# realphongha/UDP-Pose

Measured on AMD Instinct MI355X. Metric: images/sec HRNet-W32 256x192 (infer+decode), higher is better.
Workload: dtype f16x2 (split fp16 hi+lo operands = 22 bits, 3 fp16 MFMAs per product, fp32 accumulate); 1 GPU; w32 256x192 f16x2 inference, batch=64 per GPU, flip-test on, DARK decode (forward on 2N images + flip fuse + udp_decode_gaussian); global_batch=64, parallelism=replicas x1 (no data-path collective), weights=seeded synthetic, BN stats calibrated (tests/golden/bn_calib_w32_gaussian.npz)

## Files before the change

udp-pose_amd/csrc/conv_ws.hip:

```cpp
#include "conv_dev.h"

namespace udp {

template <int NB>
struct ResH2 {
  u32x4 hi[NB / 2], lo[NB / 2];
};
template <int NB>
__device__ __forceinline__ void load_res_h2(ResH2<NB>& o, __amdgpu_buffer_rsrc_t r, unsigned voff, unsigned lo_off) {
#pragma unroll
  for (int h = 0; h < NB / 2; ++h) {
    o.hi[h] = __builtin_amdgcn_raw_buffer_load_b128(r, voff + 16 * h, 0, UDP_H2_RES_AUX);
    o.lo[h] = __builtin_amdgcn_raw_buffer_load_b128(r, voff + lo_off + 16 * h, 0, UDP_H2_RES_AUX);
  }
}
template <int NB>
__device__ __forceinline__ void add_res_h2(f32x4 (&v)[NB], const ResH2<NB>& o) {
#pragma unroll
  for (int h = 0; h < NB / 2; ++h) h2_add8(v[2 * h], v[2 * h + 1], __builtin_bit_cast(f16x8, o.hi[h]), __builtin_bit_cast(f16x8, o.lo[h]));
}

template <int KS, int STRIDE, int PB, int CP, bool NCHW, bool OUT2 = false, int HS = 0>
__device__ __forceinline__ void conv_ws_body(const ConvParams& p, const int tile_id, const int cby) {
  using T = H2;
  constexpr int CK = 32, ESZ = 2, NB = 2, NW = 4;
  constexpr int PAD = KS / 2, TAPS = KS * KS;
  extern __shared__ __attribute__((aligned(16))) unsigned char smem[];

  UDP_STAMP(0);
  const int tid = threadIdx.x;
  const int lane = tid & 63;
  const int wave = __builtin_amdgcn_readfirstlane(tid >> 6);
  const int li = lane & 15;
  const int kg = lane >> 4;
  const int cp = wave % CP, pg = wave / CP;

  int t = tile_id;
  const int tx = t % p.tiles_x;
  t /= p.tiles_x;
  const int ty = t % p.tiles_y;
  const int n0 = (t / p.tiles_y) * p.G;
  const int y0 = ty * p.R;
  const int x0 = tx * p.TW;

  const int IH = p.IH, IW = p.IW;
  const int npix_in = p.G * IH * IW;
  const int in_groups = (npix_in + 15) >> 4;
  const int in_bytes = in_groups * 16 * ROWB;
  const int stage_bytes = 2 * in_bytes;
  const int nchunks = (p.Cin + CK - 1) / CK;
  const bool ragged = (p.Cin % CK) != 0;
  const int RT = p.R * p.TW;
  const int M = p.G * RT;
  const unsigned inpb = (unsigned)p.in_pitch * ESZ * 2;
  const unsigned outpb = (unsigned)p.out_pitch * ESZ * 2, respb = (unsigned)p.res_pitch * ESZ * 2;
  const unsigned in_lo = (unsigned)p.in_pitch * ESZ;
  const unsigned out_lo = (unsigned)p.out_pitch * ESZ, res_lo = (unsigned)p.res_pitch * ESZ;

  const unsigned out_pix = (unsigned)p.N * p.Hout * p.Wout;
  const __amdgpu_buffer_rsrc_t r_in = __builtin_amdgcn_make_buffer_rsrc(
      const_cast<void*>(p.in), 0, (unsigned)p.N * p.Hin * p.Win * inpb, 0x00020000);
  const unsigned npairs = (unsigned)p.CoutPad >> 5;
  const __amdgpu_buffer_rsrc_t r_w = __builtin_amdgcn_make_buffer_rsrc(
      const_cast<void*>(p.wgt), 0, (unsigned)TAPS * nchunks * npairs * 4096u, 0x00020000);
#if UDP_WS_DBG & 32
  const bool dbg_nost = nchunks == 1;
#else
  constexpr bool dbg_nost = false;
#endif
#if UDP_WS_DBG & 64
  const bool dbg_nores = nchunks == 1;
#else
  constexpr bool dbg_nores = false;
#endif
  const __amdgpu_buffer_rsrc_t r_out = __builtin_amdgcn_make_buffer_rsrc(
      p.out, 0, (!p.out || dbg_nost) ? 0 : NCHW ? out_pix * p.Cout * 4 : out_pix * outpb, 0x00020000);
  const __amdgpu_buffer_rsrc_t r_bias = __builtin_amdgcn_make_buffer_rsrc(
      const_cast<float*>(p.bias), 0, (unsigned)p.CoutPad * 4u, 0x00020000);
  const __amdgpu_buffer_rsrc_t r_res = __builtin_amdgcn_make_buffer_rsrc(
      const_cast<void*>(p.res), 0, (p.res && !dbg_nores) ? out_pix * respb : 0, 0x00020000);

  const int cwave = (cby * CP + cp) * 32;
  const int cbase = cwave + 8 * kg;
  const unsigned wvoff = (unsigned)lane * 16u;
  const unsigned wpair = (unsigned)(cby * CP + cp) * 4096u;
  constexpr int AD = UDP_WS_AD;
  f16x8 ah[AD][NB], al[AD][NB];
  const int nsteps = nchunks * TAPS;
  auto load_a = [&](int s, f16x8 (&h)[NB], f16x8 (&l)[NB]) __attribute__((always_inline)) {
    const int c = s / TAPS, tap = s - c * TAPS;
    const unsigned soff = (unsigned)(tap * nchunks + c) * (npairs * 4096u) + wpair;
#pragma unroll
    for (int nb = 0; nb < NB; ++nb) {
      h[nb] = __builtin_bit_cast(f16x8, __builtin_amdgcn_raw_buffer_load_b128(r_w, wvoff + 2048u * nb, soff, 0));
      l[nb] = __builtin_bit_cast(f16x8, __builtin_amdgcn_raw_buffer_load_b128(r_w, wvoff + 2048u * nb + 1024u, soff, 0));
    }
  };

#pragma unroll
  for (int k = 0; k < AD - 1; ++k) load_a(k < nsteps ? k : nsteps - 1, ah[k], al[k]);
  f32x4 bias[NB];
#pragma unroll
  for (int nb = 0; nb < NB; ++nb)
    bias[nb] = __builtin_bit_cast(f32x4, __builtin_amdgcn_raw_buffer_load_b128(r_bias, (unsigned)(cbase + 4 * nb) * 4u, 0, 0));

  const int srow = lane >> 2, spart = lane & 3;
  const int gy0 = y0 * STRIDE - PAD, gx0 = x0 * STRIDE - PAD;
  unsigned src_off[MAXG];
#pragma unroll
  for (int i = 0; i < MAXG; ++i) {
    unsigned off = kOobOff;
    if ((wave + NW * i) * 16 < npix_in) {
      const int row = (wave + NW * i) * 16 + srow;
      const int tmp = fdiv20(row, p.mIW);
      const int ix = row - (int)__umul24(tmp, IW);
      const int g = fdiv20(tmp, p.mIH);
      const int iy = tmp - (int)__umul24(g, IH);
      const int n = n0 + g, gy = gy0 + iy, gx = gx0 + ix;
      const bool ok = row < npix_in && n < p.N && (unsigned)gy < (unsigned)p.Hin && (unsigned)gx < (unsigned)p.Win;
      const unsigned pix = __umul24(__umul24(n, p.Hin) + gy, p.Win) + gx;
      off = ok ? pix * inpb + p.in_coff * ESZ + ((spart ^ swz<T>(row)) << 4) : kOobOff;
    }
    src_off[i] = off;
  }
  auto stage = [&](int c, unsigned char* sb) __attribute__((always_inline)) {
    const unsigned coff = (unsigned)c * (CK * ESZ);
    const bool cut = ragged && c == nchunks - 1;
    const int parts_left = (p.Cin - c * CK) / 8;
#pragma unroll
    for (int i = 0; i < MAXG; ++i) {
      const int gidx = wave + NW * i;
      if (gidx < in_groups) {
        unsigned off = src_off[i] + coff;
        if (cut && (spart ^ swz<T>(gidx * 16 + srow)) >= parts_left) off = kOobOff;
        blds16(r_in, off, sb + gidx * (16 * ROWB));
        blds16(r_in, off + in_lo, sb + in_bytes + gidx * (16 * ROWB));
      }
    }
  };

  UDP_STAMP(1);
  stage(0, smem);

  int prow[PB], opix[PB], ocrd[PB];
#pragma unroll
  for (int i = 0; i < PB; ++i) {
    const int m0 = (pg * PB + i) * 16 + li;
    const int m = m0 < M ? m0 : M - 1;
    const int g = fdiv20(m, p.mRT);
    const int rem = m - (int)__umul24(g, RT);
    const int r = fdiv20(rem, p.mTW);
    const int x = rem - (int)__umul24(r, p.TW);
    prow[i] = (int)__umul24(__umul24(g, IH) + r * STRIDE, IW) + x * STRIDE;
    const int n = n0 + g, y = y0 + r, xo = x0 + x;
    const bool ok = m0 < M && n < p.N && y < p.Hout && xo < p.Wout && (NCHW || cbase < p.Cout);
    const unsigned pix = __umul24(__umul24(n, p.Hout) + y, p.Wout) + xo;
    opix[i] = ok ? (int)pix : -1;
    ocrd[i] = ok ? (y | (xo << 10) | (n << 20)) : -1;
  }

  const float winv = __builtin_ldexpf(1.f, -p.wexp);
  f32x4 acc[PB][NB];
#pragma unroll
  for (int i = 0; i < PB; ++i)
#pragma unroll
    for (int nb = 0; nb < NB; ++nb) acc[i][nb] = f32x4{0.f, 0.f, 0.f, 0.f};

  constexpr int NR = NCHW ? 0 : PB * NB;
  ResH2<NB> rres[NCHW ? 1 : PB];
  __builtin_amdgcn_sched_barrier(0);
  asm volatile("" ::: "memory");
  if constexpr (!NCHW) {
#pragma unroll
    for (int i = 0; i < PB; ++i)
      load_res_h2(rres[i], r_res, opix[i] >= 0 ? (unsigned)opix[i] * respb + (p.res_coff + cbase) * ESZ : kOobOff, res_lo);
  }
  asm volatile("" ::: "memory");
  __builtin_amdgcn_sched_barrier(0);

  UDP_STAMP(2);
  int c = 0, tap = 0;
  const unsigned char* sb = smem;
  auto step = [&](auto BUFC, int s) __attribute__((always_inline)) {
    constexpr int BUF = decltype(BUFC)::value;
#if !(UDP_WS_DBG & 1)
    load_a(s + AD - 1 < nsteps ? s + AD - 1 : nsteps - 1, ah[(BUF + AD - 1) % AD], al[(BUF + AD - 1) % AD]);
#endif
    if (tap == 0) {
      if (c == 1) UDP_STAMP(9);
      if (c == 2) UDP_STAMP(11);
      if (c == 4) UDP_STAMP(13);
      bool refill = false;
      if constexpr (STRIDE == 2 || OUT2) refill = p.sbuf && c > 0;
      if (refill) {
        __syncthreads();
        stage(c, smem);
        asm volatile("s_waitcnt vmcnt(0)" ::: "memory");
        __syncthreads();
        sb = smem;
      } else {
        if (s == 0)
          asm volatile("s_waitcnt vmcnt(%0)" ::"n"(2 * NB + NR) : "memory");
        else
          asm volatile("s_waitcnt vmcnt(%0)" ::"n"(2 * NB) : "memory");
        if (s == 0) UDP_STAMP(3);
        __syncthreads();
        if (s == 0) UDP_STAMP(4);
        if (c == 1) UDP_STAMP(10);
        if (c == 2) UDP_STAMP(12);
        if (c == 4) UDP_STAMP(14);
#if !(UDP_WS_DBG & 4)
        if (c + 1 < nchunks && !((STRIDE == 2 || OUT2) && p.sbuf)) stage(c + 1, smem + ((c + 1) & 1) * stage_bytes);
#endif
        sb = smem + (c & 1) * stage_bytes;
      }
    }
    f16x8 a2[NB];
#pragma unroll
    for (int nb = 0; nb < NB; ++nb) a2[nb] = ah[BUF][nb] * (_Float16)0x1p-11f;
    const int tap_rows = KS == 1 ? 0 : (tap / KS) * IW + tap % KS;
    f16x8 xh[3], xl[3];
    auto load_b = [&](int i, f16x8& h, f16x8& l) __attribute__((always_inline)) {
      const int row = prow[i] + tap_rows;
      const unsigned char* q = sb + row * ROWB + ((kg ^ swz<T>(row)) << 4);
      h = *reinterpret_cast<const f16x8*>(q);
      l = *reinterpret_cast<const f16x8*>(q + in_bytes);
    };
    load_b(0, xh[0], xl[0]);
    if (PB > 1) load_b(1, xh[1], xl[1]);
#pragma unroll
    for (int i = 0; i < PB; ++i) {
#if !(UDP_WS_DBG & 2)
      if (i + 2 < PB) load_b(i + 2, xh[(i + 2) % 3], xl[(i + 2) % 3]);
#endif
      __builtin_amdgcn_sched_barrier(0);
#if UDP_WS_DBG & 16
      acc[i][0] = __builtin_amdgcn_mfma_f32_16x16x32_f16(ah[BUF][0] + al[BUF][1] + a2[0] + a2[1], xh[i % 3] + xl[i % 3], acc[i][0], 0, 0, 0);
#else
#pragma unroll
      for (int nb = 0; nb < NB; ++nb) acc[i][nb] = __builtin_amdgcn_mfma_f32_16x16x32_f16(ah[BUF][nb], xh[i % 3], acc[i][nb], 0, 0, 0);
#pragma unroll
      for (int nb = 0; nb < NB; ++nb) acc[i][nb] = __builtin_amdgcn_mfma_f32_16x16x32_f16(al[BUF][nb], xh[i % 3], acc[i][nb], 0, 0, 0);
#pragma unroll
      for (int nb = 0; nb < NB; ++nb) acc[i][nb] = __builtin_amdgcn_mfma_f32_16x16x32_f16(a2[nb], xl[i % 3], acc[i][nb], 0, 0, 0);
#endif
    }
    if (++tap == TAPS) {
      tap = 0;
      ++c;
    }
  };
  for (int s = 0; s < nsteps; s += AD) {
    step(std::integral_constant<int, 0>{}, s);
    if (s + 1 < nsteps) step(std::integral_constant<int, 1>{}, s + 1);
    if (s + 2 < nsteps) step(std::integral_constant<int, 2>{}, s + 2);
    if constexpr (AD > 3) if (s + 3 < nsteps) step(std::integral_constant<int, 3>{}, s + 3);
    if constexpr (AD > 4) if (s + 4 < nsteps) step(std::integral_constant<int, 4>{}, s + 4);
    if constexpr (AD > 5) if (s + 5 < nsteps) step(std::integral_constant<int, 5>{}, s + 5);
  }
  UDP_STAMP(5);
#pragma unroll
  for (int i = 0; i < PB; ++i) {
#pragma unroll
    for (int nb = 0; nb < NB; ++nb)
#pragma unroll
      for (int q = 0; q < 4; ++q) acc[i][nb][q] = __builtin_fmaf(acc[i][nb][q], winv, bias[nb][q]);
    if constexpr (!NCHW) add_res_h2(acc[i], rres[i]);
  }

#pragma unroll
  for (int i = 0; i < PB; ++i) {
    f32x4 v[NB];
#pragma unroll
    for (int nb = 0; nb < NB; ++nb) v[nb] = acc[i][nb];
    if constexpr (NCHW) {
      const int crd = ocrd[i];
      const int y = crd & 1023, xo = (crd >> 10) & 1023, n = crd >> 20;
      const unsigned hw = __umul24(p.Hout, p.Wout);
      const unsigned base = __umul24(__umul24(__umul24(n, p.Cout), p.Hout) + y, p.Wout) + xo;
#pragma unroll
      for (int nb = 0; nb < NB; ++nb)
#pragma unroll
        for (int q = 0; q < 4; ++q) {
          const int cc = cbase + 4 * nb + q;
          float f = v[nb][q];
          if (p.relu) f = f > 0.f ? f : 0.f;
          const unsigned off = (crd >= 0 && cc < p.Cout) ? (base + cc * hw) * 4u : kOobOff;
          __builtin_amdgcn_raw_buffer_store_b32(__builtin_bit_cast(unsigned, f), r_out, off, 0, 0);
        }
    } else {
      const unsigned ooff = opix[i] >= 0 ? (unsigned)opix[i] * outpb + (p.out_coff + cbase) * ESZ : kOobOff;
      if (p.nup) {
        const int crd = ocrd[i];
        const int y = crd & 1023, xo = (crd >> 10) & 1023, n = crd >> 20;
#pragma unroll
        for (int u = 0; u < 3; ++u) {
          if (u < p.nup) {
            const int sh = p.up_shift[u];
            const long up_pix = ((long)(n * (p.Hout >> sh) + (y >> sh)) * (p.Wout >> sh) + (xo >> sh));
            if (crd >= 0)
              add_vec<T, NB>(v, reinterpret_cast<const unsigned char*>(p.up[u]) + (up_pix * p.Cout * 2 + cbase) * ESZ, p.Cout * ESZ);
          }
        }
      }
      if constexpr (HS) {
#pragma unroll
        for (int nb = 0; nb < NB; ++nb)
#pragma unroll
          for (int q = 0; q < 4; ++q) v[nb][q] = act_hs<HS>(v[nb][q]);
      } else
      if (p.relu) {
#pragma unroll
        for (int nb = 0; nb < NB; ++nb)
#pragma unroll
          for (int q = 0; q < 4; ++q) v[nb][q] = v[nb][q] > 0.f ? v[nb][q] : 0.f;
      }
      store_vec_buf<T, NB>(r_out, ooff, out_lo, v);
      if (OUT2 && p.nout2) {
        f16x8 sh, sl;
        h2_split8(v[0], v[1], sh, sl);
        f32x4 vr[NB];
#pragma unroll
        for (int q = 0; q < 4; ++q) {
          vr[0][q] = (float)sh[q] + (float)sl[q] * kLoInv;
          vr[1][q] = (float)sh[4 + q] + (float)sl[4 + q] * kLoInv;
        }
#pragma unroll
        for (int u = 0; u < 2; ++u) {
          if (u < p.nout2 && opix[i] >= 0) {
            const size_t px = (size_t)opix[i];
            const _Float16* a = reinterpret_cast<const _Float16*>(p.add2[u]) + px * (2 * (size_t)p.add2_pitch[u]) + p.add2_coff[u] + cbase;
            const f16x8 ah8 = *reinterpret_cast<const f16x8*>(a), al8 = *reinterpret_cast<const f16x8*>(a + p.add2_pitch[u]);
            f32x4 w[NB];
#pragma unroll
            for (int q = 0; q < 4; ++q) {
              w[0][q] = ((float)ah8[q] + (float)al8[q] * kLoInv) + vr[0][q];
              w[1][q] = ((float)ah8[4 + q] + (float)al8[4 + q] * kLoInv) + vr[1][q];
            }
            f16x8 oh, ol;
            h2_split8(w[0], w[1], oh, ol);
            _Float16* o2 = reinterpret_cast<_Float16*>(p.out2[u]) + px * (2 * (size_t)p.out2_pitch[u]) + p.out2_coff[u] + cbase;
            *reinterpret_cast<f16x8*>(o2) = oh;
            *reinterpret_cast<f16x8*>(o2 + p.out2_pitch[u]) = ol;
          }
        }
      }
    }
  }
  UDP_STAMP(6);
#ifdef UDP_STAMPS
  asm volatile("s_waitcnt vmcnt(0)" ::: "memory");
  UDP_STAMP(7);
#endif
}

__host__ __device__ __forceinline__ void ws_decode(unsigned b, unsigned ntiles, unsigned nc, int& tile, int& cby) {
  if (nc == 1) {
    tile = (int)b;
    cby = 0;
    return;
  }
  const unsigned full = (ntiles >> 3) * 8u * nc;
  unsigned base = 0, width = 8, r = b;
  if (b < full) {
    const unsigned g = b / (8u * nc);
    r = b - g * 8u * nc;
    base = g * 8u;
  } else {
    r = b - full;
    base = (ntiles >> 3) * 8u;
    width = ntiles & 7u;
  }
  const unsigned c = r / width;
  cby = (int)c;
  tile = (int)(base + r - c * width);
}

template <int KS, int STRIDE, int PB, int CP, bool NCHW>
__global__ __launch_bounds__(256, 2) void conv_ws_h2_kernel(const ConvParams p) {
  int tile, cby;
  ws_decode(blockIdx.x + gridDim.x * blockIdx.y, gridDim.x, gridDim.y, tile, cby);
  conv_ws_body<KS, STRIDE, PB, CP, NCHW, KS == 3 && STRIDE == 1 && !NCHW>(p, tile, cby);
}

template <int PB, int CP, int ACT>
__global__ __launch_bounds__(256, 2) void conv_ws_hs_kernel(const ConvParams p) {
  int tile, cby;
  ws_decode(blockIdx.x + gridDim.x * blockIdx.y, gridDim.x, gridDim.y, tile, cby);
  conv_ws_body<1, 1, PB, CP, false, false, ACT>(p, tile, cby);
}

#ifndef UDP_WS_MPB
#define UDP_WS_MPB 6
#define UDP_WS_MOCC 2
#endif
template <int KS>
__global__ __launch_bounds__(256, UDP_WS_MOCC) void conv_ws_multi(const ConvMulti m) {
  const unsigned b = blockIdx.x;
  int j, tile, cby;
  int code;
  const unsigned e = __builtin_amdgcn_readfirstlane(m.tab[(b >> 3) < (unsigned)kMultiTab ? (b >> 3) : 0u]);
  if (m.tab_n) {
    j = (int)(e & 3u);
    code = 1 << ((e >> 2) & 3u);
    cby = (int)((e >> 4) & 63u);
    tile = (int)((e >> 10) + (b & 7u));
  } else {
    int sg = 0;
#pragma unroll
    for (int k = 1; k < kMultiSegs; ++k) sg += b >= m.seg_start[k];
    j = __builtin_amdgcn_readfirstlane(m.seg_mem[sg]);
    const unsigned r = __builtin_amdgcn_readfirstlane(b - m.seg_start[sg] + m.seg_first[sg]);
    ws_decode(r, m.tiles[j], m.ncby[j], tile, cby);
    tile = __builtin_amdgcn_readfirstlane(tile);
    cby = __builtin_amdgcn_readfirstlane(cby);
    code = m.code[j];
  }
  switch (code) {
    case 1: conv_ws_body<KS, 1, UDP_WS_MPB, 1, false>(m.p[j], tile, (int)cby); break;
    case 2: conv_ws_body<KS, 1, UDP_WS_MPB, 2, false>(m.p[j], tile, (int)cby); break;
    default: conv_ws_body<KS, 1, UDP_WS_MPB, 4, false>(m.p[j], tile, (int)cby); break;
  }
}

template <int KS, int STRIDE, int PB, int CP, bool NCHW>
static int describe_ws_one(const ConvParams& p, size_t lds, Launch* out) {
  static bool attr_set = false;
  const void* kern = reinterpret_cast<const void*>(&conv_ws_h2_kernel<KS, STRIDE, PB, CP, NCHW>);
  if (!attr_set) {
    UDP_HIP_CHECK(hipFuncSetAttribute(kern, hipFuncAttributeMaxDynamicSharedMemorySize, 160 * 1024));
    attr_set = true;
  }
  out->fn = kern;
  out->grid = dim3(p.ntiles, p.CoutPad / (CP * 32));
  out->block = dim3(256);
  out->lds = (unsigned)lds;
  out->p = p;
  return UDP_OK;
}
template <int KS, int STRIDE, bool NCHW>
static int describe_ws_pb(const ConvParams& p, int pb, int cp, size_t lds, Launch* out) {
#define UDP_WS(B, C) \
  if (pb == B && cp == C) return describe_ws_one<KS, STRIDE, B, C, NCHW>(p, lds, out);
  UDP_WS(2, 1) UDP_WS(3, 1) UDP_WS(4, 1) UDP_WS(6, 1) UDP_WS(2, 2) UDP_WS(3, 2) UDP_WS(4, 2) UDP_WS(6, 2)
  UDP_WS(2, 4) UDP_WS(3, 4) UDP_WS(4, 4) UDP_WS(6, 4)
#undef UDP_WS
  return 1;
}
template <int PB, int CP, int ACT>
static int describe_ws_hs_one(const ConvParams& p, size_t lds, Launch* out) {
  static bool attr_set = false;
  const void* kern = reinterpret_cast<const void*>(&conv_ws_hs_kernel<PB, CP, ACT>);
  if (!attr_set) {
    UDP_HIP_CHECK(hipFuncSetAttribute(kern, hipFuncAttributeMaxDynamicSharedMemorySize, 160 * 1024));
    attr_set = true;
  }
  out->fn = kern;
  out->grid = dim3(p.ntiles, p.CoutPad / (CP * 32));
  out->block = dim3(256);
  out->lds = (unsigned)lds;
  out->p = p;
  return UDP_OK;
}
static int describe_ws_hs(const ConvParams& p, int pb, int cp, size_t lds, Launch* out) {
#define UDP_WS(B, C) \
  if (pb == B && cp == C) return p.relu == UDP_ACT_SILU ? describe_ws_hs_one<B, C, UDP_ACT_SILU>(p, lds, out) : describe_ws_hs_one<B, C, UDP_ACT_HSWISH>(p, lds, out);
  UDP_WS(2, 1) UDP_WS(3, 1) UDP_WS(4, 1) UDP_WS(6, 1) UDP_WS(2, 2) UDP_WS(3, 2) UDP_WS(4, 2) UDP_WS(6, 2)
  UDP_WS(2, 4) UDP_WS(3, 4) UDP_WS(4, 4) UDP_WS(6, 4)
#undef UDP_WS
  return 1;
}
struct WsTile {
  int cp, pb, G, R, TW, wgs, sbuf;
  size_t lds;
};
static bool ws_tile(const ConvParams& p, int ks, int stride, int cp, int pb, WsTile* t, bool own_launch) {
  const int pg = 4 / cp;
  const int maxM = 16 * pb * pg;
  bool have = false;
  double best_util = 0.0;
  for (int split = 1; split <= 4 || !have; ++split) {
    if (split > 8) break;
    const int TW = ceil_div(p.Wout, split);
    if (TW > 64 || TW > maxM || (have && TW < 8)) continue;
    int maxR = maxM / TW;
    if (maxR > p.Hout) maxR = p.Hout;
    int R = largest_divisor_leq(p.Hout, maxR);
    if (R * 2 <= maxR) R = maxR;
    int G = 1;
    if (R == p.Hout && TW == p.Wout) {
      G = maxM / (R * TW);
      if (G > p.N) G = p.N;
      if (G < 1) G = 1;
    }
    auto npix = [&](int g, int r) { return g * ((r - 1) * stride + ks) * ((TW - 1) * stride + ks); };
    while (npix(G, R) > MAXG * 64 && G > 1) --G;
    while (npix(G, R) > MAXG * 64 && R > 1) R = (R + 1) / 2;
    if (npix(G, R) > MAXG * 64) continue;
    int nstage = ceil_div(p.Cin, 32) > 1 ? 2 : 1;
    size_t lds = (size_t)((npix(G, R) + 15) / 16) * 16 * ROWB * 2 * nstage;
    static const int sbuf_mode = getenv("UDP_POSE_WS_SBUF") == nullptr ? 1 : atoi(getenv("UDP_POSE_WS_SBUF"));
    const bool sbuf_kernel = stride == 2 || (ks == 3 && own_launch && sbuf_mode != 2);
    const bool sbuf = sbuf_kernel && nstage == 2 && lds > 80 * 1024 && lds / 2 <= 80 * 1024 && sbuf_mode != 0;
    if (sbuf) {
      nstage = 1;
      lds /= 2;
    }
    if (lds > 160 * 1024) continue;
    const int need = ceil_div(ceil_div(G * R * TW, 16), pg);
    if (need > pb) continue;
    const int pbe = need <= 2 ? 2 : need <= 3 ? 3 : need <= 4 ? 4 : 6;
    const int tiles = ceil_div(p.N, G) * ceil_div(p.Hout, R) * ceil_div(p.Wout, TW);
    const double util = (double)p.N * p.Hout * p.Wout / ((double)tiles * 16 * pbe * pg) *
                        ((double)G * R * TW * stride * stride / (double)npix(G, R));
    if (!have || util > best_util + 0.05) {
      have = true;
      best_util = util;
      t->cp = cp;
      t->pb = pbe;
      t->G = G;
      t->R = R;
      t->TW = TW;
      t->lds = lds;
      t->sbuf = sbuf ? 1 : 0;
      t->wgs = tiles * (p.CoutPad / (cp * 32));
    }
  }
  return have;
}

static long g_ws_fill_wgs = 512;
void ws_set_fill_wgs(long wgs) { g_ws_fill_wgs = wgs; }

int describe_conv_ws(ConvParams p, int ks, int stride, Launch* out, bool grouped) {
  if (p.relu >= UDP_ACT_HSWISH && (ks != 1 || stride != 1 || p.out_nchw_f32 || p.res || p.nup || p.nout2 || grouped))
    return fail(UDP_ERR_UNSUPPORTED, "hard-swish / SiLU (activation codes 2, 4): plain 1x1 stride-1 NHWC convs on their own launch only");
  if ((stride != 1 && stride != 2) || (ks != 3 && ks != 1) || (p.out_nchw_f32 && stride != 1))
    return fail(UDP_ERR_UNSUPPORTED, "fragment-major weights (wfmt 1): conv ks=%d stride=%d nchw_out=%d has no weight-stationary kernel",
                ks, stride, p.out_nchw_f32);
  auto knob = [](const char* name, long dflt) {
    const char* v = getenv(name);
    return v ? atol(v) : dflt;
  };
  const int pairs = p.CoutPad / 32;
  const int force_cp = (int)knob("UDP_POSE_WS_CP", 0), force_pb = (int)knob("UDP_POSE_WS_PB", 0);
  const long min_wgs = grouped ? 0 : knob("UDP_POSE_WS_MINWGS", g_ws_fill_wgs);
  WsTile best{}, t{};
  bool have = false;
  for (int pb : {6, 4, 3, 2}) {
    for (int cp : {4, 2, 1}) {
      if (pairs % cp || (force_cp && cp != force_cp) || (force_pb && pb != force_pb)) continue;
      if (grouped && stride == 1 && UDP_WS_MPB != 6 && pb != UDP_WS_MPB) continue;
      if (!ws_tile(p, ks, stride, cp, pb, &t, !grouped && !p.out_nchw_f32)) continue;
      const bool fills = t.wgs >= min_wgs, best_fills = have && best.wgs >= min_wgs;
      if (!have || (!best_fills && (fills || t.wgs > best.wgs))) {
        best = t;
        have = true;
      }
    }
  }
  if (!have) return fail(UDP_ERR_UNSUPPORTED, "weight-stationary conv: no tile for %dx%d C%d->%d", p.Hout, p.Wout, p.Cin, p.Cout);
  p.G = best.G;
  p.R = best.R;
  p.TW = best.TW;
  p.sbuf = best.sbuf;
  p.IH = (p.R - 1) * stride + ks;
  p.IW = (p.TW - 1) * stride + ks;
  p.tiles_x = ceil_div(p.Wout, p.TW);
  p.tiles_y = ceil_div(p.Hout, p.R);
  auto magic = [](int d) { return (unsigned)(((1u << 20) + (unsigned)d - 1) / (unsigned)d); };
  p.mIW = magic(p.IW);
  p.mIH = magic(p.IH);
  p.mRT = magic(p.R * p.TW);
  p.mTW = magic(p.TW);
  p.ntiles = ceil_div(p.N, p.G) * p.tiles_y * p.tiles_x;
  if (getenv("UDP_POSE_DEBUG_TILES"))
    fprintf(stderr, "ws conv k%d s%d %dx%d C%d->%d: G=%d R=%d TW=%d CP=%d PB=%d lds=%zu%s wgs=%d\n", ks, stride, p.Hout, p.Wout, p.Cin,
            p.Cout, p.G, p.R, p.TW, best.cp, best.pb, best.lds, best.sbuf ? " (one stage buffer)" : "", best.wgs);
  int rc = 1;
  if (ks == 3 && stride == 1 && !p.out_nchw_f32) rc = describe_ws_pb<3, 1, false>(p, best.pb, best.cp, best.lds, out);
  if (ks == 3 && stride == 1 && p.out_nchw_f32) rc = describe_ws_pb<3, 1, true>(p, best.pb, best.cp, best.lds, out);
  if (ks == 3 && stride == 2) rc = describe_ws_pb<3, 2, false>(p, best.pb, best.cp, best.lds, out);
  if (ks == 1 && stride == 1 && !p.out_nchw_f32)
    rc = p.relu >= UDP_ACT_HSWISH ? describe_ws_hs(p, best.pb, best.cp, best.lds, out) : describe_ws_pb<1, 1, false>(p, best.pb, best.cp, best.lds, out);
  if (ks == 1 && stride == 1 && p.out_nchw_f32) rc = describe_ws_pb<1, 1, true>(p, best.pb, best.cp, best.lds, out);
  if (ks == 1 && stride == 2) rc = describe_ws_pb<1, 2, false>(p, best.pb, best.cp, best.lds, out);
  if (rc == 1) return fail(UDP_ERR_UNSUPPORTED, "weight-stationary conv: no kernel for PB=%d CP=%d", best.pb, best.cp);
  if (rc == UDP_OK && p.nout2 && !(ks == 3 && stride == 1))
    return fail(UDP_ERR_UNSUPPORTED, "second outputs: 3x3 stride-1 convs only");
  if (rc == UDP_OK && grouped && best.pb == UDP_WS_MPB && stride == 1 && !p.nout2) {
    out->groupable = 300 + ks * 10 + 6;
    out->ws_cp = best.cp;
  }
  return rc;
}

static void ws_order(ConvMulti* m, int n) {
  struct Seg {
    unsigned start, first, cnt;
    int mem;
  };
  unsigned cnt_of[4];
  unsigned total = 0;
  for (int j = 0; j < n; ++j) {
    cnt_of[j] = (j + 1 < n ? m->start[j + 1] : m->start[4]) - m->start[j];
    total += cnt_of[j];
  }
  const char* mode = getenv("UDP_POSE_WS_ORDER");
  const bool lpt = mode && strcmp(mode, "lpt") == 0;
  const unsigned bias = getenv("UDP_POSE_WS_BIAS") ? (unsigned)atoi(getenv("UDP_POSE_WS_BIAS")) : 125u;
  auto build = [&](unsigned g) {
    std::vector<Seg> segs;
    unsigned lo[4] = {0, 0, 0, 0};
    unsigned at = 0;
    auto take = [&](int j, unsigned cnt) {
      if (cnt > cnt_of[j] - lo[j]) cnt = cnt_of[j] - lo[j];
      if (!cnt) return;
      if (!segs.empty() && segs.back().mem == j && segs.back().first + segs.back().cnt == lo[j])
        segs.back().cnt += cnt;
      else
        segs.push_back({at, lo[j], cnt, j});
      lo[j] += cnt;
      at += cnt;
    };
    if (!lpt) {
      const unsigned nb = cnt_of[n - 1];
      const unsigned na = total - nb;
      unsigned ta = 0, tb = 0;
      while (ta < na && tb < nb) {
        if ((unsigned long long)ta * nb * 100ull <= (unsigned long long)tb * na * bias) {
          int j = 0;
          while (lo[j] == cnt_of[j]) ++j;
          const unsigned c = cnt_of[j] - lo[j] < g ? cnt_of[j] - lo[j] : g;
          take(j, c);
          ta += c;
        } else {
          const unsigned c = nb - tb < g ? nb - tb : g;
          take(n - 1, c);
          tb += c;
        }
      }
    }
    for (int j = 0; j < n; ++j) take(j, cnt_of[j] - lo[j]);
    return segs;
  };
  unsigned g = getenv("UDP_POSE_WS_G") ? (unsigned)atoi(getenv("UDP_POSE_WS_G")) : 32u;
  if (g < 8 || g % 8) g = 32;
  std::vector<Seg> segs = build(g);
  m->tab_n = 0;
  bool ok = total % 8 == 0 && total / 8 <= (unsigned)kMultiTab && getenv("UDP_POSE_WS_NOTAB") == nullptr;
  for (int j = 0; j < n && ok; ++j)
    ok = m->tiles[j] % 8 == 0 && m->ncby[j] <= 64 && m->tiles[j] < (1u << 22) && (m->code[j] == 1 || m->code[j] == 2 || m->code[j] == 4);
  for (size_t k = 0; k < segs.size() && ok; ++k) ok = segs[k].start % 8 == 0 && segs[k].first % 8 == 0;
  if (ok) {
    for (const Seg& sg : segs) {
      const int j = sg.mem;
      for (unsigned b = sg.start; b < sg.start + sg.cnt; b += 8) {
        int tile, cby;
        ws_decode(b - sg.start + sg.first, m->tiles[j], m->ncby[j], tile, cby);
        const unsigned cl = m->code[j] == 1 ? 0u : m->code[j] == 2 ? 1u : 2u;
        m->tab[b >> 3] = (unsigned)j | (cl << 2) | ((unsigned)cby << 4) | ((unsigned)tile << 10);
      }
    }
    m->tab_n = total / 8;
  }
  while (segs.size() > (size_t)kMultiSegs) {
    g += 8;
    segs = build(g);
  }
  for (int k = 0; k < kMultiSegs; ++k) {
    const bool have = (size_t)k < segs.size();
    m->seg_start[k] = have ? segs[k].start : 0xFFFFFFFFu;
    m->seg_first[k] = have ? segs[k].first : 0;
    m->seg_mem[k] = have ? segs[k].mem : 0;
  }
}

extern "C" int udp_debug_multi_order(const unsigned* tiles, const unsigned* ncby, const int* code, int n, unsigned cap,
                                     unsigned* out_member, unsigned* out_tile, unsigned* out_cby, int* used_table) {
  if (!tiles || !ncby || !code || n < 1 || n > 4 || !out_member || !out_tile || !out_cby) return -1;
  static ConvMulti m;
  memset(&m, 0, sizeof(m));
  unsigned total = 0;
  for (int j = 0; j < n; ++j) {
    m.start[j] = total;
    m.tiles[j] = tiles[j];
    m.ncby[j] = ncby[j];
    m.code[j] = code[j];
    total += tiles[j] * ncby[j];
  }
  for (int j = n; j < 5; ++j) m.start[j] = j < 4 ? 0xFFFFFFFFu : total;
  m.start[4] = total;
  for (int j = n; j < 4; ++j) m.tiles[j] = m.ncby[j] = 1;
  if (total > cap) return -1;
  ws_order(&m, n);
  if (used_table) *used_table = m.tab_n != 0;
  for (unsigned b = 0; b < total; ++b) {
    int j, tile, cby;
    if (m.tab_n) {
      const unsigned e = m.tab[b >> 3];
      j = (int)(e & 3u);
      if ((1 << ((e >> 2) & 3u)) != m.code[j]) return -1;
      cby = (int)((e >> 4) & 63u);
      tile = (int)((e >> 10) + (b & 7u));
    } else {
      int sg = 0;
      for (int k = 1; k < kMultiSegs; ++k) sg += b >= m.seg_start[k];
      j = m.seg_mem[sg];
      ws_decode(b - m.seg_start[sg] + m.seg_first[sg], m.tiles[j], m.ncby[j], tile, cby);
    }
    out_member[b] = (unsigned)j;
    out_tile[b] = (unsigned)tile;
    out_cby[b] = (unsigned)cby;
  }
  return (int)total;
}

int describe_ws_multi(const Launch* members, int n, ConvMulti* m, Launch* out) {
  static bool ws_attr_set = false;
  const void* wk[2] = {reinterpret_cast<const void*>(&conv_ws_multi<3>), reinterpret_cast<const void*>(&conv_ws_multi<1>)};
  if (!ws_attr_set) {
    for (const void* k : wk) UDP_HIP_CHECK(hipFuncSetAttribute(k, hipFuncAttributeMaxDynamicSharedMemorySize, 160 * 1024));
    ws_attr_set = true;
  }
  memset(m, 0, sizeof(*m));
  unsigned total = 0, lds = 0;
  for (int j = 0; j < n; ++j) {
    if (members[j].groupable != members[0].groupable) return fail(UDP_ERR_ARG, "describe_multi: mixed weight-stationary members");
    m->p[j] = members[j].p;
    m->start[j] = total;
    m->tiles[j] = members[j].grid.x;
    m->ncby[j] = members[j].grid.y;
    m->code[j] = members[j].ws_cp;
    total += members[j].grid.x * members[j].grid.y;
    if (members[j].lds > lds) lds = members[j].lds;
  }
  for (int j = n; j < 5; ++j) m->start[j] = j < 4 ? 0xFFFFFFFFu : total;
  for (int j = n; j < 4; ++j) m->tiles[j] = m->ncby[j] = 1;
  ws_order(m, n);
  out->fn = wk[members[0].groupable / 10 % 10 == 3 ? 0 : 1];
  out->grid = dim3(total);
  out->block = dim3(256);
  out->lds = lds;
  out->groupable = 0;
  return UDP_OK;
}

#ifdef UDP_STAMPS
int ws_set_stamps(unsigned long long* dev_buf) {
  UDP_HIP_CHECK(hipMemcpyToSymbol(HIP_SYMBOL(g_stamps), &dev_buf, sizeof(dev_buf)));
  return UDP_OK;
}
extern "C" int udp_debug_set_stamps_ws(unsigned long long* dev_buf) { return ws_set_stamps(dev_buf); }
#endif

template <int NCH, int PB, int RD, bool LDSW>
__global__ __launch_bounds__(LDSW ? 512 : 256) __attribute__((amdgpu_waves_per_eu(2))) void conv_chain_kernel(const ConvParams p) {
  using T = H2;
  constexpr int ESZ = 2, NB = 2, Q = 2;
  constexpr int NWAVES = LDSW ? 8 : 4;
  constexpr int AD = LDSW ? 2 : 3;
  extern __shared__ __attribute__((aligned(16))) unsigned char smem[];
  const int lane = threadIdx.x & 63, wave = __builtin_amdgcn_readfirstlane(threadIdx.x >> 6);
  const int li = lane & 15, kg = lane >> 4;
  const unsigned npix = (unsigned)p.N * p.Hout * p.Wout;
  constexpr int NP = 8;
  const int cout2 = p.up_shift[0];
  const unsigned inpb = (unsigned)p.in_pitch * ESZ * 2, outpb = (unsigned)p.out_pitch * ESZ * 2, respb = (unsigned)p.res_pitch * ESZ * 2;
  const unsigned zpb = (unsigned)cout2 * ESZ * 2;
  const unsigned in_lo = (unsigned)p.in_pitch * ESZ, out_lo = (unsigned)p.out_pitch * ESZ, res_lo = (unsigned)p.res_pitch * ESZ;
  const unsigned z_lo = (unsigned)cout2 * ESZ;
  const __amdgpu_buffer_rsrc_t r_in = __builtin_amdgcn_make_buffer_rsrc(const_cast<void*>(p.in), 0, (p.sbuf & 8) ? 0 : npix * inpb, 0x00020000);
  const __amdgpu_buffer_rsrc_t r_w = __builtin_amdgcn_make_buffer_rsrc(const_cast<void*>(p.wgt), 0, (p.sbuf & 1) ? 0 : (unsigned)NCH * NP * 4096u, 0x00020000);
  const __amdgpu_buffer_rsrc_t r_w2 = __builtin_amdgcn_make_buffer_rsrc(const_cast<void*>(p.wgt2), 0, (p.sbuf & 1) ? 0 : (unsigned)NP * Q * 4096u, 0x00020000);
  const __amdgpu_buffer_rsrc_t r_bias = __builtin_amdgcn_make_buffer_rsrc(const_cast<float*>(p.bias), 0, (unsigned)p.CoutPad * 4u, 0x00020000);
  const __amdgpu_buffer_rsrc_t r_bias2 = __builtin_amdgcn_make_buffer_rsrc(const_cast<float*>(p.bias2), 0, (unsigned)cout2 * 4u, 0x00020000);
  const __amdgpu_buffer_rsrc_t r_res = __builtin_amdgcn_make_buffer_rsrc(const_cast<void*>(p.res), 0, (p.res && !(p.sbuf & 4)) ? npix * respb : 0, 0x00020000);
  const __amdgpu_buffer_rsrc_t r_out = __builtin_amdgcn_make_buffer_rsrc(p.out, 0, (p.sbuf & 2) ? 0 : npix * outpb, 0x00020000);
  const __amdgpu_buffer_rsrc_t r_z = __builtin_amdgcn_make_buffer_rsrc(const_cast<void*>(p.up[0]), 0, (p.sbuf & 2) ? 0 : npix * zpb, 0x00020000);
  const float winv = __builtin_ldexpf(1.f, -p.wexp), winv2 = __builtin_ldexpf(1.f, -p.up_shift[1]);
  const unsigned wvoff = (unsigned)lane * 16u;

  constexpr unsigned kW1 = (unsigned)NCH * 8 * 4096u, kBias = kW1 + 8u * Q * 4096u;
  if constexpr (LDSW) {
    for (unsigned blk = wave; blk < kBias / 1024u; blk += NWAVES) {
      const bool first = blk * 1024u < kW1;
      blds16(first ? r_w : r_w2, (first ? blk * 1024u : blk * 1024u - kW1) + wvoff, smem + blk * 1024u);
    }
    float* sbias = reinterpret_cast<float*>(smem + kBias);
    if (threadIdx.x < 256 + 64) sbias[threadIdx.x] = threadIdx.x < 256 ? p.bias[threadIdx.x] : p.bias2[threadIdx.x - 256];
    asm volatile("s_waitcnt vmcnt(0)" ::: "memory");
    __syncthreads();
  }
  const unsigned ngroups = (npix + PB * 16 - 1) / (PB * 16);
  for (unsigned grp = (unsigned)blockIdx.x * NWAVES + wave; grp < ngroups; grp += LDSW ? gridDim.x * NWAVES : ngroups) {
  unsigned wv = wvoff;
  int kgl = kg;
  if constexpr (LDSW) {
    asm volatile("" : "+v"(wv));
    asm volatile("" : "+v"(kgl));
  }
  unsigned pix[PB];
  bool ok[PB];
#pragma unroll
  for (int i = 0; i < PB; ++i) {
    pix[i] = grp * (PB * 16) + i * 16 + li;
    ok[i] = pix[i] < npix;
  }
  f16x8 xh[PB][NCH], xl[PB][NCH];
#pragma unroll
  for (int i = 0; i < PB; ++i)
#pragma unroll
    for (int c = 0; c < NCH; ++c) {
      const unsigned off = ok[i] ? pix[i] * inpb + (unsigned)(p.in_coff + 32 * c + 8 * kgl) * ESZ : kOobOff;
      xh[i][c] = __builtin_bit_cast(f16x8, __builtin_amdgcn_raw_buffer_load_b128(r_in, off, 0, 0));
      xl[i][c] = __builtin_bit_cast(f16x8, __builtin_amdgcn_raw_buffer_load_b128(r_in, off + in_lo, 0, 0));
    }
  constexpr int S = NCH + Q;
  f16x8 ah[AD][NB], al[AD][NB];
  auto load_a = [&](int pr, int st, f16x8 (&h)[NB], f16x8 (&l)[NB]) __attribute__((always_inline)) {
    const bool first = st < NCH;
    const unsigned soff = first ? (unsigned)(st * NP + pr) * 4096u : (unsigned)(pr * Q + (st - NCH)) * 4096u;
#pragma unroll
    for (int nb = 0; nb < NB; ++nb) {
      if constexpr (LDSW) {
        const unsigned char* q = smem + (first ? 0u : kW1) + soff + wv + 2048u * nb;
        h[nb] = *reinterpret_cast<const f16x8*>(q);
        l[nb] = *reinterpret_cast<const f16x8*>(q + 1024);
      } else {
        h[nb] = __builtin_bit_cast(f16x8, __builtin_amdgcn_raw_buffer_load_b128(first ? r_w : r_w2, wv + 2048u * nb, soff, 0));
        l[nb] = __builtin_bit_cast(f16x8, __builtin_amdgcn_raw_buffer_load_b128(first ? r_w : r_w2, wv + 2048u * nb + 1024u, soff, 0));
      }
    }
  };
  ResH2<NB> rres[RD][PB];
  auto load_res = [&](int pr, ResH2<NB> (&r)[PB]) __attribute__((always_inline)) {
#pragma unroll
    for (int i = 0; i < PB; ++i)
      load_res_h2(r[i], r_res, ok[i] ? pix[i] * respb + (unsigned)(p.res_coff + 32 * pr + 8 * kgl) * ESZ : kOobOff, res_lo);
  };
#pragma unroll
  for (int k = 0; k < RD - 1; ++k) load_res(k, rres[k]);
  load_a(0, 0, ah[0], al[0]);
  if constexpr (AD > 2) load_a(0, 1, ah[1], al[1]);

  f32x4 acc2[PB][Q][NB];
#pragma unroll
  for (int i = 0; i < PB; ++i)
#pragma unroll
    for (int q = 0; q < Q; ++q)
#pragma unroll
      for (int nb = 0; nb < NB; ++nb) acc2[i][q][nb] = f32x4{0.f, 0.f, 0.f, 0.f};

  auto mfma3 = [&](f32x4 (&acc)[NB], const f16x8 (&h)[NB], const f16x8 (&l)[NB], const f16x8 (&a2)[NB], const f16x8 bh, const f16x8 bl)
      __attribute__((always_inline)) {
#pragma unroll
        for (int nb = 0; nb < NB; ++nb) acc[nb] = __builtin_amdgcn_mfma_f32_16x16x32_f16(h[nb], bh, acc[nb], 0, 0, 0);
#pragma unroll
        for (int nb = 0; nb < NB; ++nb) acc[nb] = __builtin_amdgcn_mfma_f32_16x16x32_f16(l[nb], bh, acc[nb], 0, 0, 0);
#pragma unroll
        for (int nb = 0; nb < NB; ++nb) acc[nb] = __builtin_amdgcn_mfma_f32_16x16x32_f16(a2[nb], bl, acc[nb], 0, 0, 0);
      };

  auto pair_body = [&](auto KC) __attribute__((always_inline)) {
    constexpr int pr = decltype(KC)::value, BUF0 = (pr * S) % AD, SIDE = pr % RD;
    if constexpr (pr + RD - 1 < NP) load_res(pr + RD - 1, rres[(SIDE + RD - 1) % RD]);
    f32x4 bias[NB];
#pragma unroll
    for (int nb = 0; nb < NB; ++nb) {
      if constexpr (LDSW)
        bias[nb] = *reinterpret_cast<const f32x4*>(smem + kBias + (unsigned)(32 * pr + 8 * kgl + 4 * nb) * 4u);
      else
        bias[nb] = __builtin_bit_cast(f32x4, __builtin_amdgcn_raw_buffer_load_b128(r_bias, (unsigned)(32 * pr + 8 * kgl + 4 * nb) * 4u, 0, 0));
    }
    f32x4 acc[PB][NB];
#pragma unroll
    for (int i = 0; i < PB; ++i)
#pragma unroll
      for (int nb = 0; nb < NB; ++nb) acc[i][nb] = f32x4{0.f, 0.f, 0.f, 0.f};
    f16x8 yh[PB], yl[PB];
#pragma unroll
    for (int st = 0; st < S; ++st) {
      constexpr int dummy = 0;
      (void)dummy;
      const int buf = (BUF0 + st) % AD;
      {
// ... 109 lines not shown
```

Measured before the change: 8117 images/s.

## Add PB=8 weight-stationary conv variant with late residual loads and peeled tail

Adds a PB=8 (eight pixel blocks per wave group, CP=1) variant of the weight-stationary 3x3 stride-1 conv for grouped launches with an odd number of channel pairs. It is offered in the tile search and the multi-kernel dispatch table. The main loop now peels the last three steps, moving the residual loads into that tail so they no longer occupy registers and vmcnt slots through the whole K loop. The variant also drops the nup coordinate registers. These changes aim at more reuse of each weight fragment per MFMA and lower register pressure, at the cost of tighter tile constraints (exact fit, LDS at most 80KB) and more template code paths. The residual loads may now be exposed latency at the end of the loop.

```diff
diff --git a/udp-pose_amd/csrc/conv_ws.hip b/udp-pose_amd/csrc/conv_ws.hip
--- a/udp-pose_amd/csrc/conv_ws.hip
+++ b/udp-pose_amd/csrc/conv_ws.hip
@@ -2,6 +2,9 @@
 
 namespace udp {
 
+#ifndef UDP_WS_LATE_RES
+#define UDP_WS_LATE_RES 1
+#endif
 template <int NB>
 struct ResH2 {
   u32x4 hi[NB / 2], lo[NB / 2];
@@ -20,7 +23,7 @@
   for (int h = 0; h < NB / 2; ++h) h2_add8(v[2 * h], v[2 * h + 1], __builtin_bit_cast(f16x8, o.hi[h]), __builtin_bit_cast(f16x8, o.lo[h]));
 }
 
-template <int KS, int STRIDE, int PB, int CP, bool NCHW, bool OUT2 = false, int HS = 0>
+template <int KS, int STRIDE, int PB, int CP, bool NCHW, bool OUT2 = false, int HS = 0, bool NUP = true>
 __device__ __forceinline__ void conv_ws_body(const ConvParams& p, const int tile_id, const int cby) {
   using T = H2;
   constexpr int CK = 32, ESZ = 2, NB = 2, NW = 4;
@@ -142,7 +145,7 @@
   UDP_STAMP(1);
   stage(0, smem);
 
-  int prow[PB], opix[PB], ocrd[PB];
+  int prow[PB], opix[PB], ocrd[NCHW || NUP ? PB : 1];
 #pragma unroll
   for (int i = 0; i < PB; ++i) {
     const int m0 = (pg * PB + i) * 16 + li;
@@ -156,7 +159,7 @@
     const bool ok = m0 < M && n < p.N && y < p.Hout && xo < p.Wout && (NCHW || cbase < p.Cout);
     const unsigned pix = __umul24(__umul24(n, p.Hout) + y, p.Wout) + xo;
     opix[i] = ok ? (int)pix : -1;
-    ocrd[i] = ok ? (y | (xo << 10) | (n << 20)) : -1;
+    if constexpr (NCHW || NUP) ocrd[i] = ok ? (y | (xo << 10) | (n << 20)) : -1;
   }
 
   const float winv = __builtin_ldexpf(1.f, -p.wexp);
@@ -166,27 +169,35 @@
 #pragma unroll
     for (int nb = 0; nb < NB; ++nb) acc[i][nb] = f32x4{0.f, 0.f, 0.f, 0.f};
 
+  constexpr bool LATE = UDP_WS_LATE_RES && KS == 3 && STRIDE == 1 && !NCHW && AD == 3;
   constexpr int NR = NCHW ? 0 : PB * NB;
   ResH2<NB> rres[NCHW ? 1 : PB];
-  __builtin_amdgcn_sched_barrier(0);
-  asm volatile("" ::: "memory");
-  if constexpr (!NCHW) {
-#pragma unroll
-    for (int i = 0; i < PB; ++i)
+  constexpr int RSPLIT = LATE && PB > 6 ? PB / 2 : PB;
+  auto load_res = [&](auto I0, auto I1) __attribute__((always_inline)) {
+    __builtin_amdgcn_sched_barrier(0);
+    asm volatile("" ::: "memory");
+#pragma unroll
+    for (int i = decltype(I0)::value; i < (NCHW ? 0 : decltype(I1)::value); ++i)
       load_res_h2(rres[i], r_res, opix[i] >= 0 ? (unsigned)opix[i] * respb + (p.res_coff + cbase) * ESZ : kOobOff, res_lo);
-  }
-  asm volatile("" ::: "memory");
-  __builtin_amdgcn_sched_barrier(0);
+    asm volatile("" ::: "memory");
+    __builtin_amdgcn_sched_barrier(0);
+  };
+  if constexpr (!LATE) load_res(std::integral_constant<int, 0>{}, std::integral_constant<int, PB>{});
 
   UDP_STAMP(2);
   int c = 0, tap = 0;
   const unsigned char* sb = smem;
-  auto step = [&](auto BUFC, int s) __attribute__((always_inline)) {
-    constexpr int BUF = decltype(BUFC)::value;
+  auto step = [&](auto BUFC, auto TAILC, int s) __attribute__((always_inline)) {
+    constexpr int BUF = decltype(BUFC)::value, TAIL = decltype(TAILC)::value;
 #if !(UDP_WS_DBG & 1)
-    load_a(s + AD - 1 < nsteps ? s + AD - 1 : nsteps - 1, ah[(BUF + AD - 1) % AD], al[(BUF + AD - 1) % AD]);
+    if constexpr (!LATE)
+      load_a(s + AD - 1 < nsteps ? s + AD - 1 : nsteps - 1, ah[(BUF + AD - 1) % AD], al[(BUF + AD - 1) % AD]);
+    else if constexpr (TAIL <= 0)
+      load_a(s + AD - 1, ah[(BUF + AD - 1) % AD], al[(BUF + AD - 1) % AD]);
 #endif
-    if (tap == 0) {
+    if constexpr (TAIL == 0) load_res(std::integral_constant<int, 0>{}, std::integral_constant<int, RSPLIT>{});
+    if constexpr (TAIL == 1 && RSPLIT < PB) load_res(std::integral_constant<int, RSPLIT>{}, std::integral_constant<int, PB>{});
+    if (TAIL < 0 && tap == 0) {
       if (c == 1) UDP_STAMP(9);
       if (c == 2) UDP_STAMP(11);
       if (c == 4) UDP_STAMP(13);
@@ -200,7 +211,7 @@
         sb = smem;
       } else {
         if (s == 0)
-          asm volatile("s_waitcnt vmcnt(%0)" ::"n"(2 * NB + NR) : "memory");
+          asm volatile("s_waitcnt vmcnt(%0)" ::"n"(2 * NB + (LATE ? 0 : NR)) : "memory");
         else
           asm volatile("s_waitcnt vmcnt(%0)" ::"n"(2 * NB) : "memory");
         if (s == 0) UDP_STAMP(3);
@@ -218,7 +229,7 @@
     f16x8 a2[NB];
 #pragma unroll
     for (int nb = 0; nb < NB; ++nb) a2[nb] = ah[BUF][nb] * (_Float16)0x1p-11f;
-    const int tap_rows = KS == 1 ? 0 : (tap / KS) * IW + tap % KS;
+    const int tap_rows = KS == 1 ? 0 : TAIL >= 0 ? (KS - 1) * IW + TAIL : (tap / KS) * IW + tap % KS;
     f16x8 xh[3], xl[3];
     auto load_b = [&](int i, f16x8& h, f16x8& l) __attribute__((always_inline)) {
       const int row = prow[i] + tap_rows;
@@ -245,18 +256,32 @@
       for (int nb = 0; nb < NB; ++nb) acc[i][nb] = __builtin_amdgcn_mfma_f32_16x16x32_f16(a2[nb], xl[i % 3], acc[i][nb], 0, 0, 0);
 #endif
     }
-    if (++tap == TAPS) {
-      tap = 0;
-      ++c;
+    if constexpr (TAIL < 0) {
+      if (++tap == TAPS) {
+        tap = 0;
+        ++c;
+      }
     }
   };
-  for (int s = 0; s < nsteps; s += AD) {
-    step(std::integral_constant<int, 0>{}, s);
-    if (s + 1 < nsteps) step(std::integral_constant<int, 1>{}, s + 1);
-    if (s + 2 < nsteps) step(std::integral_constant<int, 2>{}, s + 2);
-    if constexpr (AD > 3) if (s + 3 < nsteps) step(std::integral_constant<int, 3>{}, s + 3);
-    if constexpr (AD > 4) if (s + 4 < nsteps) step(std::integral_constant<int, 4>{}, s + 4);
-    if constexpr (AD > 5) if (s + 5 < nsteps) step(std::integral_constant<int, 5>{}, s + 5);
+  constexpr std::integral_constant<int, -1> LOOP{};
+  if constexpr (LATE) {
+    for (int s = 0; s < nsteps - AD; s += AD) {
+      step(std::integral_constant<int, 0>{}, LOOP, s);
+      step(std::integral_constant<int, 1>{}, LOOP, s + 1);
+      step(std::integral_constant<int, 2>{}, LOOP, s + 2);
+    }
+    step(std::integral_constant<int, 0>{}, std::integral_constant<int, 0>{}, nsteps - 3);
+    step(std::integral_constant<int, 1>{}, std::integral_constant<int, 1>{}, nsteps - 2);
+    step(std::integral_constant<int, 2>{}, std::integral_constant<int, 2>{}, nsteps - 1);
+  } else {
+    for (int s = 0; s < nsteps; s += AD) {
+      step(std::integral_constant<int, 0>{}, LOOP, s);
+      if (s + 1 < nsteps) step(std::integral_constant<int, 1>{}, LOOP, s + 1);
+      if (s + 2 < nsteps) step(std::integral_constant<int, 2>{}, LOOP, s + 2);
+      if constexpr (AD > 3) if (s + 3 < nsteps) step(std::integral_constant<int, 3>{}, LOOP, s + 3);
+      if constexpr (AD > 4) if (s + 4 < nsteps) step(std::integral_constant<int, 4>{}, LOOP, s + 4);
+      if constexpr (AD > 5) if (s + 5 < nsteps) step(std::integral_constant<int, 5>{}, LOOP, s + 5);
+    }
   }
   UDP_STAMP(5);
 #pragma unroll
@@ -290,8 +315,8 @@
         }
     } else {
       const unsigned ooff = opix[i] >= 0 ? (unsigned)opix[i] * outpb + (p.out_coff + cbase) * ESZ : kOobOff;
-      if (p.nup) {
-        const int crd = ocrd[i];
+      if (NUP && p.nup) {
+        const int crd = ocrd[NUP ? i : 0];
         const int y = crd & 1023, xo = (crd >> 10) & 1023, n = crd >> 20;
 #pragma unroll
         for (int u = 0; u < 3; ++u) {
@@ -394,6 +419,8 @@
 #define UDP_WS_MPB 6
 #define UDP_WS_MOCC 2
 #endif
+constexpr int kWsCode8 = 8;
+constexpr bool kWsHave8 = UDP_WS_MPB == 6 && UDP_WS_LATE_RES && UDP_WS_AD == 3;
 template <int KS>
 __global__ __launch_bounds__(256, UDP_WS_MOCC) void conv_ws_multi(const ConvMulti m) {
   const unsigned b = blockIdx.x;
@@ -416,11 +443,21 @@
     cby = __builtin_amdgcn_readfirstlane(cby);
     code = m.code[j];
   }
+  if constexpr (KS == 3 && kWsHave8) {
+    if (code == kWsCode8) {
+      conv_ws_body<KS, 1, 8, 1, false, false, 0, false>(m.p[j], tile, (int)cby);
+      return;
+    }
+  }
   switch (code) {
     case 1: conv_ws_body<KS, 1, UDP_WS_MPB, 1, false>(m.p[j], tile, (int)cby); break;
     case 2: conv_ws_body<KS, 1, UDP_WS_MPB, 2, false>(m.p[j], tile, (int)cby); break;
     default: conv_ws_body<KS, 1, UDP_WS_MPB, 4, false>(m.p[j], tile, (int)cby); break;
   }
+}
+
+__global__ __launch_bounds__(256, 2) void conv_ws_pb8_kernel(const ConvParams p) {
+  conv_ws_body<3, 1, 8, 1, false, false, 0, false>(p, (int)blockIdx.x, (int)blockIdx.y);
 }
 
 template <int KS, int STRIDE, int PB, int CP, bool NCHW>
@@ -446,6 +483,20 @@
   UDP_WS(2, 4) UDP_WS(3, 4) UDP_WS(4, 4) UDP_WS(6, 4)
 #undef UDP_WS
   return 1;
+}
+static int describe_ws_pb8(const ConvParams& p, size_t lds, Launch* out) {
+  static bool attr_set = false;
+  const void* kern = reinterpret_cast<const void*>(&conv_ws_pb8_kernel);
+  if (!attr_set) {
+    UDP_HIP_CHECK(hipFuncSetAttribute(kern, hipFuncAttributeMaxDynamicSharedMemorySize, 160 * 1024));
+    attr_set = true;
+  }
+  out->fn = kern;
+  out->grid = dim3(p.ntiles, p.CoutPad / 32);
+  out->block = dim3(256);
+  out->lds = (unsigned)lds;
+  out->p = p;
+  return UDP_OK;
 }
 template <int PB, int CP, int ACT>
 static int describe_ws_hs_one(const ConvParams& p, size_t lds, Launch* out) {
@@ -507,9 +558,10 @@
       lds /= 2;
     }
     if (lds > 160 * 1024) continue;
+    if (pb == 8 && (G * R * TW != maxM || p.Hout % R || TW * split != p.Wout || lds > 80 * 1024)) continue;
     const int need = ceil_div(ceil_div(G * R * TW, 16), pg);
     if (need > pb) continue;
-    const int pbe = need <= 2 ? 2 : need <= 3 ? 3 : need <= 4 ? 4 : 6;
+    const int pbe = need <= 2 ? 2 : need <= 3 ? 3 : need <= 4 ? 4 : need <= 6 ? 6 : 8;
     const int tiles = ceil_div(p.N, G) * ceil_div(p.Hout, R) * ceil_div(p.Wout, TW);
     const double util = (double)p.N * p.Hout * p.Wout / ((double)tiles * 16 * pbe * pg) *
                         ((double)G * R * TW * stride * stride / (double)npix(G, R));
@@ -545,10 +597,13 @@
   const int pairs = p.CoutPad / 32;
   const int force_cp = (int)knob("UDP_POSE_WS_CP", 0), force_pb = (int)knob("UDP_POSE_WS_PB", 0);
   const long min_wgs = grouped ? 0 : knob("UDP_POSE_WS_MINWGS", g_ws_fill_wgs);
+  const bool offer8 = kWsHave8 && grouped && ks == 3 && stride == 1 && pairs % 2 == 1 && !p.out_nchw_f32 && !p.nout2 && !p.nup &&
+                      knob("UDP_POSE_WS_PB8", 1) != 0;
   WsTile best{}, t{};
   bool have = false;
-  for (int pb : {6, 4, 3, 2}) {
+  for (int pb : {8, 6, 4, 3, 2}) {
     for (int cp : {4, 2, 1}) {
+      if (pb == 8 && (!offer8 || cp != 1)) continue;
       if (pairs % cp || (force_cp && cp != force_cp) || (force_pb && pb != force_pb)) continue;
       if (grouped && stride == 1 && UDP_WS_MPB != 6 && pb != UDP_WS_MPB) continue;
       if (!ws_tile(p, ks, stride, cp, pb, &t, !grouped && !p.out_nchw_f32)) continue;
@@ -578,6 +633,9 @@
     fprintf(stderr, "ws conv k%d s%d %dx%d C%d->%d: G=%d R=%d TW=%d CP=%d PB=%d lds=%zu%s wgs=%d\n", ks, stride, p.Hout, p.Wout, p.Cin,
             p.Cout, p.G, p.R, p.TW, best.cp, best.pb, best.lds, best.sbuf ? " (one stage buffer)" : "", best.wgs);
   int rc = 1;
+  if (best.pb == 8) {
+    rc = describe_ws_pb8(p, best.lds, out);
+  } else
   if (ks == 3 && stride == 1 && !p.out_nchw_f32) rc = describe_ws_pb<3, 1, false>(p, best.pb, best.cp, best.lds, out);
   if (ks == 3 && stride == 1 && p.out_nchw_f32) rc = describe_ws_pb<3, 1, true>(p, best.pb, best.cp, best.lds, out);
   if (ks == 3 && stride == 2) rc = describe_ws_pb<3, 2, false>(p, best.pb, best.cp, best.lds, out);
@@ -588,8 +646,8 @@
   if (rc == 1) return fail(UDP_ERR_UNSUPPORTED, "weight-stationary conv: no kernel for PB=%d CP=%d", best.pb, best.cp);
   if (rc == UDP_OK && p.nout2 && !(ks == 3 && stride == 1))
     return fail(UDP_ERR_UNSUPPORTED, "second outputs: 3x3 stride-1 convs only");
-  if (rc == UDP_OK && grouped && best.pb == UDP_WS_MPB && stride == 1 && !p.nout2) {
-    out->groupable = 300 + ks * 10 + 6;
+  if (rc == UDP_OK && grouped && (best.pb == UDP_WS_MPB || best.pb == 8) && stride == 1 && !p.nout2) {
+    out->groupable = 300 + ks * 10 + (best.pb == 8 ? 8 : 6);
     out->ws_cp = best.cp;
   }
   return rc;
@@ -650,7 +708,7 @@
   m->tab_n = 0;
   bool ok = total % 8 == 0 && total / 8 <= (unsigned)kMultiTab && getenv("UDP_POSE_WS_NOTAB") == nullptr;
   for (int j = 0; j < n && ok; ++j)
-    ok = m->tiles[j] % 8 == 0 && m->ncby[j] <= 64 && m->tiles[j] < (1u << 22) && (m->code[j] == 1 || m->code[j] == 2 || m->code[j] == 4);
+    ok = m->tiles[j] % 8 == 0 && m->ncby[j] <= 64 && m->tiles[j] < (1u << 22) && (m->code[j] == 1 || m->code[j] == 2 || m->code[j] == 4 || m->code[j] == kWsCode8);
   for (size_t k = 0; k < segs.size() && ok; ++k) ok = segs[k].start % 8 == 0 && segs[k].first % 8 == 0;
   if (ok) {
     for (const Seg& sg : segs) {
@@ -658,7 +716,7 @@
       for (unsigned b = sg.start; b < sg.start + sg.cnt; b += 8) {
         int tile, cby;
         ws_decode(b - sg.start + sg.first, m->tiles[j], m->ncby[j], tile, cby);
-        const unsigned cl = m->code[j] == 1 ? 0u : m->code[j] == 2 ? 1u : 2u;
+        const unsigned cl = m->code[j] == 1 ? 0u : m->code[j] == 2 ? 1u : m->code[j] == 4 ? 2u : 3u;
         m->tab[b >> 3] = (unsigned)j | (cl << 2) | ((unsigned)cby << 4) | ((unsigned)tile << 10);
       }
     }
@@ -726,12 +784,12 @@
   memset(m, 0, sizeof(*m));
   unsigned total = 0, lds = 0;
   for (int j = 0; j < n; ++j) {
-    if (members[j].groupable != members[0].groupable) return fail(UDP_ERR_ARG, "describe_multi: mixed weight-stationary members");
+    if (members[j].groupable / 10 != members[0].groupable / 10) return fail(UDP_ERR_ARG, "describe_multi: mixed weight-stationary members");
     m->p[j] = members[j].p;
     m->start[j] = total;
     m->tiles[j] = members[j].grid.x;
     m->ncby[j] = members[j].grid.y;
-    m->code[j] = members[j].ws_cp;
+    m->code[j] = members[j].groupable % 10 == 8 ? kWsCode8 : members[j].ws_cp;
     total += members[j].grid.x * members[j].grid.y;
     if (members[j].lds > lds) lds = members[j].lds;
   }
```

New measurement: 8267 images/s, median of 6. 1.8% higher.
